# TinyMPC/tinympc-matlab

Hardware: AMD Instinct MI355X
Metric: ADMM iterations/s, batched quadrotor nx=12 nu=4 N=50 (instance-iterations/s, whole job) (higher is better)
Workload: dtype f64

## Files before the change

### __graft_entry__.py

```python
from __future__ import annotations

import hashlib
import importlib.util
import os
import re
import shutil
import subprocess
import sys

ROOT = os.path.dirname(os.path.abspath(__file__))
if ROOT not in sys.path:
    sys.path.insert(0, ROOT)
PKG_DIR = os.path.join(ROOT, "tinympc-matlab_amd")
PKG_NAME = "tinympc_matlab_amd"
CSRC = os.path.join(PKG_DIR, "csrc")
HIP_LIB = os.path.join(PKG_DIR, "libtinympc_hip.so")
ORACLE_DIR = os.path.join(ROOT, "oracle")
REFERENCE_SRC = "/root/reference/src/codegen_src"

HIP_SOURCES = ["tinympc_kernels.hip", "tinympc_precompute_rows.hip", "tinympc_solve.hip", "tinympc_solve_b.hip", "tinympc_solve_fam.hip", "tinympc_solve_adapt.hip", "tinympc_imod_a.hip", "tinympc_solve_c.hip", "tinympc_solve_d.hip", "tinympc_solve_dr.hip", "tinympc_lean_d.hip", "tinympc_lstart_d.hip", "tinympc_ltrim_d.hip", "tinympc_solve_dw.hip", "tinympc_solve_dx.hip", "tinympc_jit.hip", "tinympc_solve_m.hip", "tinympc_precompute_large.hip", "tinympc_handle.hip", "tinympc_plan.hip", "tinympc_session.hip", "tinympc_capi.hip",
               "tinympc_codegen.hip"]
HIP_LINTED = ["tinympc_precompute_rows.hip", "tinympc_solve.hip", "tinympc_solve_b.hip", "tinympc_solve_fam.hip", "tinympc_solve_adapt.hip", "tinympc_imod_a.hip",
              "tinympc_solve_c.hip", "tinympc_solve_d.hip", "tinympc_solve_dr.hip", "tinympc_lean_d.hip", "tinympc_lstart_d.hip", "tinympc_ltrim_d.hip", "tinympc_solve_dw.hip", "tinympc_solve_dx.hip"]
JIT_EMBEDDED = ["tinympc_device.h", "tinympc_sweep.h", "tinympc_fam_red.h", "tinympc_solve_d_chain.h", "tinympc_solve_dw_chain.h", "tinympc_solve_dx_chain.h",
                "tinympc_solve_e_common.h", "tinympc_solve_dwide.h", "tinympc_solve_d.hip", "tinympc_solve_dw.hip", "tinympc_solve_dx.hip", "tinympc_solve_e.hip",
                "tinympc_solve_f.hip"]
_ROCKET = ["-DTINY_JIT_NX=6", "-DTINY_JIT_NU=3", "-DTINY_JIT_N=100", "-DTINY_JIT_CT=0", "-DTINY_JIT_FAM=1"]
_ROCKET_FAM = ["-DTINY_JIT_E_NROUND=1", "-DTINY_JIT_E_NCONE=2", "-DTINY_JIT_E_CONES={0,0,2},{0,6,8}", "-DTINY_JIT_E_NLX=1", "-DTINY_JIT_E_NLU=0"]
HIP_BUILTINS = [
    ("k_builtin_e_rocket100", "tinympc_solve_e.hip",
     _ROCKET + ["-DTINY_JIT_E_WPG=8", "-DTINY_JIT_E_WPS=2", "-DTINY_JIT_E_S=13"] + _ROCKET_FAM +
     ["-DTINY_JIT_E_GC_LDS=0", "-DTINY_JIT_E_GL_LDS=0", "-DTINY_JIT_E_LX_LDS=0", "-DTINY_JIT_E_KFAM=1", "-DTINY_JIT_E_DREG=1"]),
    ("k_builtin_f_rocket100", "tinympc_solve_f.hip", _ROCKET + ["-DTINY_JIT_F_WPG=4", "-DTINY_JIT_F_S=7"] + _ROCKET_FAM + ["-DTINY_JIT_F_KFAM=1"]),
    ("k_builtin_f_rocket100_session", "tinympc_solve_f.hip", _ROCKET + ["-DTINY_JIT_F_WPG=4", "-DTINY_JIT_F_S=7"] + _ROCKET_FAM + ["-DTINY_JIT_F_KFAM=1", "-DTINY_JIT_F_SESSION=1"]),
]
_NO_FAM = ["-DTINY_JIT_E_NROUND=0", "-DTINY_JIT_E_NCONE=0", "-DTINY_JIT_E_CONES={-1,0,0}", "-DTINY_JIT_E_NLX=0", "-DTINY_JIT_E_NLU=0"]
for _name, _nx, _nu, _N, _wpg, _S in (("cartpole20", 4, 1, 20, 2, 3), ("quadrotor50", 12, 4, 50, 4, 4)):
    for _suffix, _ct, _extra in (("", 1, []), ("_var", 0, []), ("_session", 0, ["-DTINY_JIT_F_SESSION=1"])):
        HIP_BUILTINS.append(("k_builtin_f_%s%s" % (_name, _suffix), "tinympc_solve_f.hip",
                             ["-DTINY_JIT_NX=%d" % _nx, "-DTINY_JIT_NU=%d" % _nu, "-DTINY_JIT_N=%d" % _N, "-DTINY_JIT_CT=%d" % _ct, "-DTINY_JIT_FAM=0",
                              "-DTINY_JIT_F_WPG=%d" % _wpg, "-DTINY_JIT_F_S=%d" % _S] + _NO_FAM + _extra))
HIP_BUILTINS_D = [("k_builtin_d_quadrotor50_models", "tinympc_solve_d.hip",
                   ["-DTINY_JIT_NX=12", "-DTINY_JIT_NU=4", "-DTINY_JIT_N=50", "-DTINY_JIT_VREG=49", "-DTINY_JIT_WPS=1", "-DTINY_JIT_WPG=4",
                    "-DTINY_JIT_CT=1", "-DTINY_JIT_FAM=0", "-DTINY_JIT_ADAPT=0", "-DTINY_JIT_IMOD=1"])]
ALL_BUILTINS = HIP_BUILTINS + HIP_BUILTINS_D
BUILD_DIR = os.path.join(ROOT, "build", "hip")
HIP_CFLAGS = ["--offload-arch=gfx950", "-O3", "-std=c++17", "-fPIC", "-fno-gpu-rdc",
              "-Wall", "-Wno-unused-function", "-I" + os.path.join(ROOT, "include"), "-I" + CSRC, "-I" + BUILD_DIR]
HIP_LDFLAGS = ["--offload-arch=gfx950", "-shared", "-fPIC", "-fno-gpu-rdc", "-lhiprtc"]


def load_package():
    if PKG_NAME in sys.modules:
        return sys.modules[PKG_NAME]
    spec = importlib.util.spec_from_file_location(
        PKG_NAME, os.path.join(PKG_DIR, "__init__.py"), submodule_search_locations=[PKG_DIR])
# ... 292 lines not shown
```

### tinympc-matlab_amd/csrc/tinympc_device.h

```cpp
#pragma once
#ifndef __HIPCC_RTC__
#include <hip/hip_runtime.h>
#endif

namespace tinympc {

__host__ __device__ inline size_t ops_doubles(int W, int KT) { return (size_t)2 * W * KT + 3 * W; }

__host__ __device__ inline size_t table_rows(int N) { return (size_t)N + 2; }

constexpr int V_PAD = 4;
__host__ __device__ inline size_t v_rows(int N) { return (size_t)N + 1 + 2 * V_PAD; }
__host__ __device__ inline size_t tables_doubles(int W, int N) { return 3 * table_rows(N) * W + W; }

#if defined(__HIPCC__) || defined(__HIPCC_RTC__)
__device__ __forceinline__ void host_store(double *p, double v) { __hip_atomic_store(p, v, __ATOMIC_RELAXED, __HIP_MEMORY_SCOPE_SYSTEM); }
#endif

struct PrecomputeParams {
    int nx, nu;
    double rho;
    const double *A, *B, *fdyn, *Qd, *Rd;
    double *Kinf, *Pinf, *Quu_inv, *AmBKt, *APf, *BPf;
    int *info;
// ... 250 lines not shown
    double *zero;
    size_t zero_doubles;
    double *xmin, *xmax, *umin, *umax;
    size_t X, U;
    double inf;
    double *rho_inst;
    int batch;
    double rho;
    double *mail;
};
hipError_t launch_setup_init(const SetupInitParams &p, hipStream_t stream);
hipError_t launch_fill_bounds(double *xmin, double *xmax, size_t X, double *umin, double *umax, size_t U, double inf, hipStream_t stream);
hipError_t launch_reset_stats(int *istats, double *dstats, double *rho_inst, int batch, double rho, hipStream_t stream);
size_t lqr_scratch_doubles(int nx, int nu);
size_t precompute_large_scratch_doubles(int nx, int nu);
hipError_t launch_precompute_large(const PrecomputeParams &p, hipStream_t stream);
hipError_t launch_build_operators(const OperatorParams &p, hipStream_t stream);
hipError_t launch_build_tables(const TableParams &p, hipStream_t stream);
hipError_t launch_store_inst_refs(const InstRefStoreParams &p, hipStream_t stream);
hipError_t launch_build_inst_tables(const InstTableParams &p, hipStream_t stream);
hipError_t launch_fill_inst_models(const InstModelFillParams &p, hipStream_t stream);
hipError_t launch_store_inst_diag(const InstDiagParams &p, hipStream_t stream);
enum class SolveExt { Box, Families, Adaptive, InstRefs, InstBounds, InstModels };
hipError_t launch_solve_a(const SolveParams &p, SolveExt ext, int W, int KT, size_t lds_bytes, hipStream_t stream);
hipError_t launch_solve_b(const SolveParams &p, int W, int KT, size_t lds_bytes, hipStream_t stream);
size_t solve_b_lds_bytes(int nx, int nu, int N, int W);
constexpr int WAVES_PER_GROUP_B = 4;
bool solve_d_supported(int nx, int nu, int N, bool const_tables);
hipError_t launch_solve_d(const SolveParams &p, hipStream_t stream);
hipError_t launch_solve_d_refill(const SolveParams &p, hipStream_t stream);
hipError_t launch_solve_d_lean(const SolveParams &p, hipStream_t stream);
hipError_t launch_solve_d_lean_start(const SolveParams &p, hipStream_t stream);
hipError_t launch_solve_d_lean_trim(const SolveParams &p, hipStream_t stream);
int solve_d_workgroups(int nu, int N, bool const_tables, int groups);
size_t solve_d_lds_bytes(int nu, int N, bool const_tables);
int solve_d_resident_workgroups(int wpg);
int solve_d_wavefronts_per_workgroup(int nu, int N, bool const_tables);
bool solve_dw_supported(int nx, int nu, int N, bool const_tables);
hipError_t launch_solve_dw(const SolveParams &p, hipStream_t stream);
int solve_dw_workgroups(int nu, int N, int groups);
size_t solve_dw_lds_bytes(int nu, int N);
bool solve_dx_supported(int nx, int nu, int N, bool const_tables);
hipError_t launch_solve_dx(const SolveParams &p, hipStream_t stream);
int solve_dx_workgroups(int nu, int N, int groups);
size_t solve_dx_lds_bytes(int nu, int N);
hipError_t launch_solve_c(const SolveParams &p, int W, int KT, size_t lds_bytes, hipStream_t stream);
hipError_t launch_build_chunk_tables(const ChunkTableParams &p, hipStream_t stream);
size_t f_input_table_doubles(int nu, int S);
hipError_t launch_build_f_input_tables(const ChunkTableParams &p, hipStream_t stream);
void chunk_plan(int N, int *S, int *C, int *Lc);
size_t solve_c_lds_bytes(int nx, int Lc);
size_t solve_c_lds_bytes_refs(int nx, int nu, int N, int Lc);
size_t chunk_table_doubles(int nx, int Lc);
int chunk_ks(int nx);
hipError_t launch_build_adapt(const AdaptTableParams &p, hipStream_t stream);
inline hipError_t ensure_dynamic_lds(const void *fn, size_t bytes, size_t (&cache)[16]) {
    int dev = 0;
    hipError_t e = hipGetDevice(&dev);
    if (e != hipSuccess) return e;
    if (dev >= 0 && dev < 16 && cache[dev] >= bytes) return hipSuccess;
    e = hipFuncSetAttribute(fn, hipFuncAttributeMaxDynamicSharedMemorySize, (int)bytes);
    if (e == hipSuccess && dev >= 0 && dev < 16) cache[dev] = bytes;
    return e;
}

bool solve_m_supported(int nx, int nu);
// ... 32 lines not shown
```

### tinympc-matlab_amd/csrc/tinympc_plan.hip

```cpp
#include <cstring>
#include "tinympc_handle.h"

using namespace tinympc;
using namespace tinympc::host;

namespace {

void arm_completion_flag(tinympc_solver *s, SolveParams &p) {
    if (!p.host_sol) return;
    s->session_seq += 1;
    p.host_seq = (double)s->session_seq;
    s->flag_pending = true;
}

void decide_layout_d_variants(tinympc_solver *s) {
    if (!s->layout_d) return;
    if (s->d_varying < 0 && !s->tables_const()) {
        if (s->W == 16 && !s->d_jit && solve_d_supported(s->nx, s->nu, s->N, false)) {
            s->d_varying = 1;
        } else {
            s->d_varying_jit = solve_jit_supported(s->W, s->nx, s->nu, s->N, false);
            s->d_varying = s->d_varying_jit ? 1 : 0;
        }
    }
// ... 205 lines not shown
    const bool ct = s->tables_const();
    long resident;
    if (jit) resident = solve_jit_resident_wavefronts(s->W, s->nx, s->nu, s->N, ct);
    else {
        const int wpg = solve_d_wavefronts_per_workgroup(s->nu, s->N, ct);
        resident = (long)solve_d_resident_workgroups(wpg) * wpg;
    }
    const bool reachable = s->st.abs_pri_tol > 0.0 && s->st.abs_dua_tol > 0.0;
    if ((long)s->groups <= resident) return false;
    if (!reachable && mode != 1) return false;
    return !jit || solve_jit_refill_supported(s->W, s->nx, s->nu, s->N, ct);
}

static bool lean_applies(const tinympc_solver *s, const LaunchPlan &pl) {
    if (pl.kernel != KernelId::D_COMPILED || s->W != 16 || pl.adaptive || pl.families || s->zero_copy_tick || s->st.max_iter <= 0)
        return false;
    if (pl.inst_models) return false;
    if (refill_applies(s, pl)) return false;
    const char *env = getenv("TINYMPC_LEAN");
    const int mode = env ? atoi(env) : -1;
    if (mode == 0) return false;
    if (mode == 1) return true;
    const bool reachable = s->st.abs_pri_tol > 0.0 && s->st.abs_dua_tol > 0.0;
    return s->st.check_termination != 1 || !reachable;
}
static bool lean_start_applies() {
    const char *env = getenv("TINYMPC_LEAN_START");
    return !env || atoi(env) != 0;
}
static bool lean_trim_applies() {
    const char *env = getenv("TINYMPC_LEAN_TRIM");
    return lean_start_applies() && (!env || atoi(env) != 0);
}
static const char *lean_words(const tinympc_solver *s, const LaunchPlan &pl) {
    return !lean_applies(s, pl) ? "" : lean_trim_applies() ? " lean lds-start trim" : lean_start_applies() ? " lean lds-start" : " lean";
}

int launch(tinympc_solver *s, bool timed) {
    int rc;
    s->flag_pending = false;
    if ((rc = resolve_plan(s))) return rc;
    const LaunchPlan pl = current_plan(s);
    const bool fam = pl.families, adaptive = pl.adaptive;
    if (s->inst_tables() && !pl.inst_refs) {
        const bool r = s->inst.refs(), b = s->inst.bounds, m = s->inst.models;
        const char *what[3], *back[3];
        int n = 0;
        if (r) { what[n] = "per-instance references (set_x_ref_batch / set_u_ref_batch)"; back[n++] = "tinympc_set_x_ref / tinympc_set_u_ref return to shared references"; }
        if (b) { what[n] = "per-instance bounds (set_bound_constraints_batch)"; back[n++] = "tinympc_set_bound_constraints returns to shared bounds"; }
        if (m) { what[n] = "per-instance models (set_model_batch)"; back[n++] = "tinympc_clear_model_batch returns to the shared model"; }
        std::string subj, way;
        for (int i = 0; i < n; ++i) {
            subj += std::string(i == 0 ? "" : i == n - 1 ? " and " : ", ") + what[i];
            way += std::string(i == 0 ? "" : ", ") + back[i];
        }
        return fail(TINYMPC_ERR_UNSUPPORTED, "%s are not supported %s; %s", subj.c_str(),
                    s->layout_m ? "for systems with nx+nu > 64" : fam ? "with cone / linear constraint families" : "with adaptive rho", way.c_str());
    }
    if (s->refs_on_host && (adaptive || pl.inst_models)) {
        if ((rc = flush_host_refs(s))) return rc;
    }
    if ((rc = refresh_derived(s))) return rc;
    if (adaptive && fam)
        return fail(TINYMPC_ERR_UNSUPPORTED, "adaptive_rho together with cone / linear constraint families is not supported");
    if (s->layout_m && adaptive)
        return fail(TINYMPC_ERR_UNSUPPORTED, "adaptive_rho is not supported for systems with nx+nu > 64");
    if (fam && pl.kernel != KernelId::E && pl.kernel != KernelId::F && pl.kernel != KernelId::M && family_structure(s).beyond_generic())
        return fail(TINYMPC_ERR_UNSUPPORTED, "more than %d linear rows per side, %d cones or %d rounds of overlapping cones run on the run-time "
// ... 54 lines not shown
        p.dXref = s->dXref; p.dUref = s->dUref; p.Pinf = s->dPinf;
        s->refs_on_host = false;
    }
    p.adapt = s->dadapt; p.rho_inst = s->drho_inst;
    if (pl.inst_refs) {
        p.iref_lr = pl.kernel == KernelId::A ? s->inst.lr_rows() : s->inst.lrg;
        p.iref_pn = s->inst.pn;
        if (pl.kernel != KernelId::A) p.ibnd = s->inst.bndg;
        else if (pl.inst_bounds) p.ibnd = s->inst.bnd;
    }
    p.rho_min = s->st.adaptive_rho_min; p.rho_max = s->st.adaptive_rho_max; p.rho_clip = s->st.adaptive_rho_enable_clipping;
    const bool kernel_takes_cold = (pl.kernel == KernelId::D_COMPILED || pl.kernel == KernelId::D_JIT) && s->st.max_iter > 0;
    if (s->cold_state && !kernel_takes_cold && (rc = materialize_cold_state(s))) return rc;
    p.cold = s->cold_state ? 1 : 0;
    s->cold_state = false;
    if (s->st.max_iter > 0) s->sol_zero_pending = false;
    else if ((rc = materialize_zero_solution(s))) return rc;
    if (refill_applies(s, pl) && !p.x0_mirror && !p.u0_host && !p.host_sol) {
        if (!s->drefill && (rc = dalloc(s, &s->drefill, 1))) return rc;
        HIP_TRY(hipMemsetAsync(s->drefill, 0, sizeof(int), s->stream));
        p.refill_next = s->drefill;
    }
    if (timed) HIP_TRY(hipEventRecord(s->ev0, s->stream));
    switch (pl.kernel) {
        case KernelId::M:
            p.ctab = s->dctab;
            HIP_TRY(launch_solve_m(p, s->stream));
            break;
        case KernelId::D_JIT:
            HIP_TRY(launch_solve_jit(p, s->W, s->stream, pl.inst_models));
            break;
        case KernelId::D_COMPILED:
            if (lean_applies(s, pl) && !p.x0_mirror && !p.u0_host && !p.refill_next)
                HIP_TRY(lean_trim_applies()    ? launch_solve_d_lean_trim(p, s->stream)
                        : lean_start_applies() ? launch_solve_d_lean_start(p, s->stream)
                                               : launch_solve_d_lean(p, s->stream));
            else HIP_TRY(s->W == 64 ? launch_solve_dx(p, s->stream) : s->W == 32 ? launch_solve_dw(p, s->stream) : launch_solve_d(p, s->stream));
            break;
        case KernelId::E:
            p.ctab = s->dctab_e; p.chunk_len = s->e_chunk_len; p.chunk_count = s->e_wpg; p.chunk_levels = 1;
            HIP_TRY(launch_solve_e(p, s->fs, s->stream));
            break;
        case KernelId::F:
            p.ctab = s->dctab_f; p.ftab = s->dftab; p.chunk_len = s->f_chunk_len; p.chunk_count = s->f_chunks; p.chunk_levels = 4;
            arm_completion_flag(s, p);
            HIP_TRY(launch_solve_f(p, s->f_fs, s->stream));
            break;
        case KernelId::C:
            p.ctab = s->dctab; p.chunk_len = s->chunk_len; p.chunk_count = s->chunk_count; p.chunk_levels = s->chunk_levels;
            arm_completion_flag(s, p);
            HIP_TRY(launch_solve_c(p, s->W, s->KT, s->lds_bytes_c, s->stream));
            break;
        case KernelId::B:
            HIP_TRY(launch_solve_b(p, s->W, s->KT, s->lds_bytes, s->stream));
            break;
        case KernelId::A:
        case KernelId::FAM_A:
        case KernelId::ADAPT_A: {
            const SolveExt ext = pl.kernel == KernelId::FAM_A ? SolveExt::Families : pl.kernel == KernelId::ADAPT_A ? SolveExt::Adaptive
                                 : pl.inst_models ? SolveExt::InstModels : pl.inst_bounds ? SolveExt::InstBounds : pl.inst_refs ? SolveExt::InstRefs : SolveExt::Box;
            HIP_TRY(launch_solve_a(p, ext, s->W, s->KT, s->lds_bytes_a, s->stream));
            break;
        }
    }
    if (timed) HIP_TRY(hipEventRecord(s->ev1, s->stream));
    return TINYMPC_OK;
}
// ... 77 lines not shown
```

### tinympc-matlab_amd/csrc/tinympc_solve_d.hip

```cpp
#if defined(TINY_BUILTIN) && !defined(TINY_JIT)
#define TINY_JIT 1
#endif
#ifndef TINY_JIT
#include <atomic>
#endif
#include <type_traits>

#include "tinympc_device.h"
#include "tinympc_sweep.h"

#ifndef TINY_REFILL
#if defined(TINY_JIT_REFILL) && TINY_JIT_REFILL
#define TINY_REFILL 1
#else
#define TINY_REFILL 0
#endif
#endif

#ifndef TINY_LEAN
#define TINY_LEAN 0
#endif
#if TINY_LEAN && (TINY_REFILL || defined(TINY_JIT))
#error "TINY_LEAN: compiled-in plain kernels only"
#endif
#ifndef TINY_LEAN_START
#define TINY_LEAN_START 0
#endif
#if TINY_LEAN_START && !TINY_LEAN
#error "TINY_LEAN_START: a variant of the lean kernels"
#endif
#if TINY_LEAN_START && !defined(TINY_LEAN_NO_LDS_START)
#define TINY_LDS_START 1
#else
#define TINY_LDS_START 0
#endif
#if TINY_LEAN_START && !defined(TINY_LEAN_NO_HOIST)
#define TINY_LEAN_HOIST 1
#else
#define TINY_LEAN_HOIST 0
#endif
#ifndef TINY_LEAN_TRIM
#define TINY_LEAN_TRIM 0
#endif
#if TINY_LEAN_TRIM && !(TINY_LEAN_START && TINY_LEAN_HOIST && TINY_LDS_START)
#error "TINY_LEAN_TRIM: a variant of the lean-start kernels (LDS starts and hoisted control)"
#endif
#if TINY_LEAN_TRIM && !defined(TINY_TRIM_NO_DSTORE)
#define TINY_TRIM_DSTORE 1
#define D_DUMP_DOUBLES(nu) (2 * 4 * (nu))
#else
#define TINY_TRIM_DSTORE 0
#endif

#define TINY_STR2(x) #x
#define TINY_STR(x) TINY_STR2(x)
namespace tinympc {
template <int NX, int NU>
struct DStep;
}

#ifdef TINY_JIT
#define D_NX TINY_JIT_NX
#define D_NU TINY_JIT_NU
#include "tinympc_solve_d_chain.h"
#else
#define D_NX 12
#define D_NU 4
#include "tinympc_solve_d_chain.h"
#define D_NX 4
#define D_NU 1
#include "tinympc_solve_d_chain.h"
#endif

namespace tinympc {

template <int I, int E, class F>
__device__ __forceinline__ void static_for(F &&f) {
    if constexpr (I < E) {
        f(std::integral_constant<int, I>{});
        static_for<I + 1, E>(f);
    }
}

constexpr int D_OPS_DOUBLES = 2 * 16 * 16;
// ... 35 lines not shown
    const int want = ns > D_VREG_MAX ? ns - D_VREG_MAX : 0;
    return want <= vlmax ? want : -1;
}
__host__ __device__ constexpr size_t d_lds_bytes(int nu, int N, bool ct, int wpg, int vl, bool fam = false, bool adapt = false, bool imod = false) {
    return sizeof(double) * ((size_t)(imod ? 0 : D_OPS_DOUBLES + D_START_DOUBLES) + (ct ? 0 : d_tab_doubles(N)) + (fam ? D_FAM_DOUBLES : 0) + (adapt ? D_ADAPT_DOUBLES : 0) +
#if TINY_TRIM_DSTORE
                             (size_t)wpg * (vl * 64 + D_DUMP_DOUBLES(nu) + d_d_doubles(nu, N) + (imod ? D_IMOD_WAVE_DOUBLES : 0)));
#else
                             (size_t)wpg * (vl * 64 + d_d_doubles(nu, N) + (imod ? D_IMOD_WAVE_DOUBLES : 0)));
#endif
}

__device__ __forceinline__ unsigned lds_addr(const double *p) { return lds_address(p); }
template <int OFF>
__device__ __forceinline__ double lds_read_async(unsigned addr) {
    return lds_read_issued_here<OFF>(addr);
}
template <int OFF>
__device__ __forceinline__ void lds_write_async(unsigned addr, double v) {
    static_assert(OFF >= 0 && OFF < 65536, "ds offset field is 16 bits");
    asm volatile("ds_write_b64 %0, %1 offset:%2" ::"v"(addr), "v"(v), "n"(OFF) : "memory");
}
template <int OFF>
__device__ __forceinline__ void lds_write_masked(unsigned addr, double v, unsigned long long mask) {
    static_assert(OFF >= 0 && OFF < 65536, "ds offset field is 16 bits");
    unsigned long long saved;
    asm volatile("s_and_saveexec_b64 %[sv], %[m]\n\t"
                 "ds_write_b64 %[a], %[v] offset:%[o]\n\t"
                 "s_mov_b64 exec, %[sv]"
                 : [sv] "=&s"(saved)
                 : [m] "s"(mask), [a] "v"(addr), [v] "v"(v), [o] "n"(OFF)
                 : "memory", "scc");
}
__device__ __forceinline__ void lds_wait() {
    lds_reads_landed();
    asm volatile("" ::: "memory");
}
__device__ __forceinline__ void lds_wait_ops(double (&m)[16]) {
    lds_reads_landed();
#ifdef TINY_D_NO_OPS_WAIT
    asm volatile("" ::: "memory");
#else
    asm volatile(""
                 : "+v"(m[0]), "+v"(m[1]), "+v"(m[2]), "+v"(m[3]), "+v"(m[4]), "+v"(m[5]), "+v"(m[6]), "+v"(m[7]), "+v"(m[8]), "+v"(m[9]),
                   "+v"(m[10]), "+v"(m[11]), "+v"(m[12]), "+v"(m[13]), "+v"(m[14]), "+v"(m[15])
                 :
                 : "memory");
#endif
}

__device__ __forceinline__ bool wave_may_converge_d(unsigned long long bad, unsigned long long live) {
    int any = 0;
#pragma unroll
    for (int j = 0; j < 4; ++j) {
        const unsigned b = (unsigned)(bad >> (j * 16)) & 0xffffu, l = (unsigned)(live >> (j * 16)) & 0xffffu;
        any |= (int)(l != 0u) & (int)(b == 0u);
    }
    return any != 0;
}
#ifdef TINY_D_NO_RARE
#define TINY_RARE(c) (c)
#else
#define TINY_RARE(c) __builtin_expect(!!(c), 0)
#endif

#if TINY_REFILL
// ... 516 lines not shown
#endif
            }
#if TINY_REFILL
            if (TINY_RARE(may) && is_x && active) gV1u[REFILL ? row_offset(cur) : (unsigned)lane] = V0;
#else
            if (TINY_RARE(may) && is_x && active) gV1u[(unsigned)lane] = V0;
#endif
            V0 = snew;
        }
        if constexpr (FAM) {
            double gcn, gln;
            (void)families(x0v, GC0, GL0, gcn, gln);
            if (is_x) {
                GC0 = gcn;
                GL0 = gln;
            }
        }
        double xcur = x0v;
        double dcur = lds_read_async<0>(aD), vcur = 0.0;
#if TINY_LEAN
        if constexpr (VL > 0 && !LEANI) vcur = lds_read_async<0>(aV);
#else
        if constexpr (VL > 0) vcur = lds_read_async<0>(aV);
#endif
        double locur = lo_c, hicur = hi_c;
        if constexpr (!CT) {
            locur = lds_read_async<W * 8>(aT);
            hicur = lds_read_async<(TOFF + W) * 8>(aT);
        }
        lds_wait_ops(m);
#if TINY_LDS_START
        double acur = 0.0;
#endif
        auto fstep = [&](auto S) {
            constexpr int q = decltype(S)::value;
            double dn = 0.0, vn = 0.0, lon = lo_c, hin = hi_c;
            if constexpr (q + 1 < NS) dn = lds_read_async<(q + 1) * DS * 8>(aD);
#if TINY_LEAN
            if constexpr (q + 1 < VL && !LEANI) vn = lds_read_async<(q + 1) * 512>(aV);
#else
            if constexpr (q + 1 < VL) vn = lds_read_async<(q + 1) * 512>(aV);
#endif
            if constexpr (!CT && q + 1 < NS) {
                lon = lds_read_async<(q + 2) * W * 8>(aT);
                hin = lds_read_async<(TOFF + (q + 2) * W) * 8>(aT);
            }
#if TINY_LDS_START
            static_assert(K0, "step 0 starts from c0");
            double an = 0.0;
            if constexpr (LEANI && q + 1 < NS) an = lds_read_issued_here<0>(aC);
#endif
            const double xprev = xcur;
            double snew_q;
#if TINY_LEAN
            if constexpr (LEANI) {
                if constexpr (q >= VL) {
                    if constexpr (K0 && q == 0) xcur = Step::fwd_reg0_nores(dcur, m, c0, locur, hicur, G[q], Vr[q - VL]);
#if TINY_LDS_START
                    else xcur = Step::fwd_reg_start(xcur, dcur, m, acur, locur, hicur, G[q], Vr[q - VL]);
#else
                    else xcur = Step::fwd_reg_nores(xcur, dcur, m, cf, locur, hicur, G[q], Vr[q - VL]);
#endif
                    snew_q = Vr[q - VL];
                } else {
                    double vnew;
                    if constexpr (K0 && q == 0) xcur = Step::fwd_lds0_nores(dcur, m, c0, locur, hicur, G[q], vnew);
#if TINY_LDS_START
                    else xcur = Step::fwd_lds_start(xcur, dcur, m, acur, locur, hicur, G[q], vnew);
#else
                    else xcur = Step::fwd_lds_nores(xcur, dcur, m, cf, locur, hicur, G[q], vnew);
#endif
                    lds_write_async<q * 512>(aV, vnew);
                    snew_q = vnew;
                }
            } else
#endif
            if constexpr (q >= VL) {
                if constexpr (K0 && q == 0) xcur = Step::fwd_reg0(dcur, m, c0, locur, hicur, G[q], Vr[q - VL], pri, dua);
                else xcur = Step::fwd_reg(xcur, dcur, m, cf, locur, hicur, G[q], Vr[q - VL], pri, dua);
                snew_q = Vr[q - VL];
            } else {
                double vnew;
                if constexpr (K0 && q == 0) xcur = Step::fwd_lds0(dcur, m, c0, locur, hicur, G[q], vcur, vnew, pri, dua);
                else xcur = Step::fwd_lds(xcur, dcur, m, cf, locur, hicur, G[q], vcur, vnew, pri, dua);
                lds_write_async<q * 512>(aV, vnew);
                snew_q = vnew;
            }
            if constexpr (ADAPT) {
                if (adapt) {
                    const double gnew = G[q], out = xcur;
                    const double t = group_matvec<W, 16>(mtr, is_x ? gnew : 0.0, 0.0);
                    const double dgx = dgr * (is_x ? xprev : out);
                    const double aty = is_x ? (t - gprev) : (gnew + t);
                    a_dn = fmax(fmax(a_dn, fabs(dgx)), fabs(aty));
                    a_dr = fmax(a_dr, fabs(2.0 * dgx + aty));
                    a_pr = fmax(a_pr, fabs(is_x ? snew_q : (out - snew_q)));
                    a_pn = fmax(fmax(a_pn, fabs(snew_q)), is_x ? 0.0 : fabs(out));
                    gprev = gnew;
                }
            }
            if constexpr (FAM) {
                double gcn, gln;
                const double l = families(xcur, GCr[q], GLr[q], gcn, gln);
                if (row_ok) {
                    GCr[q] = gcn;
                    GLr[q] = gln;
                    LX[q] = l;
                }
            }
            dcur = dn;
            vcur = vn;
#if TINY_LDS_START
            acur = an;
#endif
            if constexpr (!CT) {
                locur = lon;
                hicur = hin;
            }
        };
        constexpr int DF = D_FIRST < NS ? D_FIRST : NS;
        constexpr int NG = 1 + (NS - DF + D_GROUP - 1) / D_GROUP;
        static_for<0, NG>([&](auto Gi) {
            constexpr int s0 = Gi.value == 0 ? 0 : DF + (Gi.value - 1) * D_GROUP;
            constexpr int s1 = Gi.value == 0 ? DF : ((s0 + D_GROUP < NS) ? s0 + D_GROUP : NS);
            if (TINY_RARE(may)) {
                if constexpr (s0 > 0) {
                    if (!adapt) {
                        const bool bad = !((pri < p.abs_pri_tol) && (dua * rho < p.abs_dua_tol));
#if TINY_REFILL
                        may = __builtin_amdgcn_readfirstlane((int)wave_may_converge_d(__ballot(bad), __ballot(REFILL ? chk : active))) != 0;
#else
                        may = __builtin_amdgcn_readfirstlane((int)wave_may_converge_d(__ballot(bad), __ballot(active))) != 0;
#endif
                    }
                }
                if (TINY_RARE(may)) {
#if TINY_REFILL
                    unsigned vo = REFILL ? row_offset(cur) + (unsigned)(koff * 64) : voff;
#else
                    unsigned vo = voff;
#endif
                    double *base = gV1u;
                    asm volatile("" : "+v"(vo), "+s"(base));
                    if (active) static_for<s0, s1>([&](auto S) { (base + S.value * 64)[vo] = vget(S); });
                }
            }
// ... 96 lines not shown
                } else if constexpr (FOLD) {
                    asm("v_add_f64 %[t], %[v1], -%[g1]\n\t"
                        "v_fma_f64 %[px], %[sc], %[t], %[lrT]\n\t"
                        "v_add_f64 %[rn], %[v2], -%[g2]\n\t"
                        "v_fma_f64 %[acc], %[rhom], %[rn], %[lrmc]"
                        : [t] "=&v"(t), [px] "=&v"(px), [acc] "=&v"(acc), [rn] "=&v"(rnext)
                        : [v1] "v"(v1), [g1] "v"(G[NS - 1]), [v2] "v"(v2), [g2] "v"(G[NS - 2]), [sc] "v"(is_x ? nrho : 1.0),
                          [lrT] "v"(is_x ? pnref : 0.0), [rhom] "v"(rhom), [lrmc] "v"(lrmc_f));
                } else {
                    asm("v_add_f64 %[t], %[v1], -%[g1]\n\t"
                        "v_fma_f64 %[px], %[nrho], %[t], %[lrT]\n\t"
                        "v_add_f64 %[t], %[v2], -%[g2]\n\t"
                        "v_fma_f64 %[acc], %[rhom], %[t], %[lrmc]\n\t"
                        "v_fma_f64 %[rn], %[nrho], %[t], %[lr]"
                        : [t] "=&v"(t), [px] "=&v"(px), [acc] "=&v"(acc), [rn] "=&v"(rnext)
                        : [v1] "v"(v1), [g1] "v"(G[NS - 1]), [v2] "v"(v2), [g2] "v"(G[NS - 2]), [nrho] "s"(nrho), [lrT] "v"(lrT),
                          [rhom] "v"(rhom), [lrmc] "v"(lrmc2), [lr] "v"(lr2));
                }
                rcur = px;
            }
            auto vreq = [&](auto S) -> double {
                if constexpr (decltype(S)::value >= VL) return Vr[decltype(S)::value - VL];
                else return lds_read_async<decltype(S)::value * 512>(aV);
            };
            double v2cur = vreq(std::integral_constant<int, (NS >= 3 ? NS - 3 : 0)>{});
            lds_wait_ops(m);
#if TINY_LEAN_HOIST
            if constexpr (LEANI) {
                asm volatile("" : "+v"(G0));
                G0 = G0 - V0;
                asm volatile("" ::"v"(G0));
            }
#endif
            static_for<0, NS - 1>([&](auto I) {
                constexpr int s = NS - 1 - I.value;
                constexpr int s2 = s >= 2 ? s - 2 : 0;
                constexpr int s3 = s >= 3 ? s - 3 : 0;
                double v2n = 0.0;
                if constexpr (s >= 2) v2n = vreq(std::integral_constant<int, s3>{});
                const double lr2 = lr_of(std::integral_constant<int, s2>{});
                const double lrmc2 = is_x ? lr2 + cb : cb;
                double a = acc, an, rn;
                if constexpr (ADAPT) Step::bwd_v(a, px, rcur, m, v2cur, G[s2], rhom_lin, lrmc2, nrho_lin, lr2, an, rn);
                else if constexpr (FOLD) Step::bwd_fold(a, px, rcur, m, v2cur, G[s2], rhom, lrmc_f, an, rn);
                else Step::bwd(a, px, rcur, m, v2cur, G[s2], rhom, lrmc2, nrho, lr2, an, rn);
#if TINY_TRIM_DSTORE
                if constexpr (NO_CTL) lds_write_async<s * DS * 8>(aDw, a);
                else lds_write_masked<s * DS * 8>(aD, a, wr_d);
#else
                lds_write_masked<s * DS * 8>(aD, a, wr_d);
#endif
                px = a;
                rcur = rnext;
                rnext = rn;
                acc = an;
                v2cur = v2n;
            });
            {
                double a = acc;
                Step::bwd_last(a, px, rcur, m);
#if TINY_TRIM_DSTORE
                if constexpr (NO_CTL) lds_write_async<0>(aDw, a);
                else lds_write_masked<0>(aD, a, wr_d);
#else
                lds_write_masked<0>(aD, a, wr_d);
#endif
            }
        }
#if TINY_LEAN
        return false;
    };
    const bool reachable = p.abs_pri_tol > 0.0 && p.abs_dua_tol > 0.0;
    const int last_check = ct > 0 ? (max_iter / ct) * ct : 0;
    for (int it = 0; max_iter > 0;) {
        int nres = max_iter + 1;
        if (ct > 0 && reachable) nres = (it / ct + 1) * ct;
        else if (last_check > it) nres = last_check;
        const int lean_end = __builtin_amdgcn_readfirstlane(nres - 1 < max_iter ? nres - 1 : max_iter);
#if TINY_LEAN_HOIST
        if (it < lean_end) {
            if (iteration(std::integral_constant<int, 2>{}, it)) break;
#if TINY_TRIM_DSTORE
            {
                const unsigned long long live = __ballot(active);
                const unsigned lm = (unsigned)(live & 1ull) | (unsigned)((live >> 15) & 2ull) | (unsigned)((live >> 30) & 4ull) | (unsigned)((live >> 45) & 8ull);
                const int first = __builtin_ctz(lm | 16u);
                const int cls = (r / NU) % 3;
                int jt = cls == 0 ? j : (j ^ 2);
                if (((lm >> jt) & 1u) == 0u) jt = first & 3;
                const unsigned dump = lds_addr(sD) + (unsigned)((jt * NU + r % NU) * 8) - (unsigned)((cls == 2 ? 2 : 1) * DS * 8);
                aDw = (is_u && active) ? aD : dump;
            }
#endif
            for (; it < lean_end; ++it) (void)iteration(std::true_type{}, it);
// ... 32 lines not shown
    }

    const double res_px = group_max<W>(is_x ? snap_pri : 0.0), res_pu = group_max<W>(is_u ? snap_pri : 0.0);
    const double rho_res = ADAPT ? snap_rho : rho;
    const double res_dx = group_max<W>(is_x ? snap_dua : 0.0) * rho_res, res_du = group_max<W>(is_u ? snap_dua : 0.0) * rho_res;

#ifdef TINY_CLOCK_STAMP
    if (p.scratch && lane == 0) {
        unsigned long long *ck = reinterpret_cast<unsigned long long *>(p.scratch) + 8 * (size_t)grp;
        ck[0] = ck_t1 - ck_t0;
        ck[1] = ck_r1 - ck_r0;
        ck[2] = ck_barrier - ck_entry;
        ck[3] = ck_r0 - ck_barrier;
        ck[4] = __builtin_amdgcn_s_memrealtime() - ck_r1;
        ck[5] = ck_entry;
        ck[6] = __builtin_amdgcn_s_memrealtime();
        ck[7] = (unsigned long long)__builtin_amdgcn_s_getreg((31 << 11) | 4) | ((unsigned long long)__builtin_amdgcn_s_getreg((3 << 11) | 20) << 32);
    }
#endif
    if (inst_ok && r == 0) {
        if constexpr (ADAPT) p.rho_inst[inst] = rho;
        p.istats[inst * 2 + 0] = it_done;
        p.istats[inst * 2 + 1] = status;
        if (res_valid) {
            p.dstats[inst * 4 + 0] = res_px;
            p.dstats[inst * 4 + 1] = res_dx;
            p.dstats[inst * 4 + 2] = res_pu;
            p.dstats[inst * 4 + 3] = res_du;
        }
    }
}

#if TINY_LEAN
#if TINY_LEAN_TRIM
#define k_admm_solve_d_lean k_admm_solve_d_lean_trim
#define k_admm_solve_d_gbnd_lean k_admm_solve_d_gbnd_lean_trim
#define launch_solve_d_lean launch_solve_d_lean_trim
static_assert(d_vl(4, 50, true, 4) == 25, "quadrotor N=50: 25 slack slots in LDS with four wavefronts per workgroup");
#elif TINY_LEAN_START
#define k_admm_solve_d_lean k_admm_solve_d_lean_start
#define k_admm_solve_d_gbnd_lean k_admm_solve_d_gbnd_lean_start
#define launch_solve_d_lean launch_solve_d_lean_start
static_assert(d_vl(4, 50, true, 4) == 25, "quadrotor N=50: 25 slack slots in LDS with four wavefronts per workgroup");
#endif
template <int NX, int NU, int N, bool CT, int WPG, int VL>
__global__ void __launch_bounds__(64 * WPG) __attribute__((amdgpu_waves_per_eu(2, 2))) k_admm_solve_d_lean(const SolveParams p) {
    extern __shared__ __attribute__((aligned(16))) double smem[];
    k_admm_solve_d_body<NX, NU, N, CT, WPG, VL>(p, smem);
}
template <int NX, int NU, int N, int WPG, int VL>
__global__ void __launch_bounds__(64 * WPG) __attribute__((amdgpu_waves_per_eu(2, 2))) k_admm_solve_d_gbnd_lean(const SolveParams p) {
    extern __shared__ __attribute__((aligned(16))) double smem[];
    k_admm_solve_d_body<NX, NU, N, true, WPG, VL, false, false, true, false, false, true>(p, smem);
}

__host__ __device__ constexpr int d_wpg(int nu, int N, bool ct) { return d_vl(nu, N, ct, 4) >= 0 ? 4 : 8; }

template <int NX, int NU, int N, bool CT>
static hipError_t launch_d_one(const SolveParams &p, hipStream_t stream) {
    constexpr int WPG = d_wpg(NU, N, CT);
    constexpr int VL = d_vl(NU, N, CT, WPG);
    if constexpr (VL < 0) {
        return hipErrorInvalidValue;
    } else {
        constexpr size_t lds = d_lds_bytes(NU, N, CT, WPG, VL);
        static size_t lds_set_l[16] = {0}, lds_set_lgoal[16] = {0};
        const int wgs = (p.groups + WPG - 1) / WPG;
// ... 230 lines not shown
```

### tinympc-matlab_amd/csrc/tinympc_solve_d_chain.h

```cpp
#if !defined(D_NX) || !defined(D_NU)
#error "define D_NX and D_NU before including tinympc_solve_d_chain.h"
#endif
#if D_NX < 1 || D_NU < 1 || D_NX + D_NU > 16
#error "layout D: 1 <= nx, 1 <= nu, nx + nu <= 16"
#endif

#ifdef TINY_CHAIN_NOALIGN
#define D_AL ""
#define D_MOV64 "v_mov_b64"
#else
#define D_AL ".p2align 3\n\t"
#ifdef TINY_CHAIN_MOV32
#define D_MOV64 "v_mov_b64"
#else
#define D_MOV64 "v_mov_b64_e64"
#endif
#endif
#if (defined(TINY_JIT) && !defined(TINY_BUILTIN)) || defined(TINY_CHAIN_NOP)
#define D_HAZ "s_nop 1\n\t" D_AL
#else
#define D_HAZ D_AL
#endif
#define D_FM_(src, i) "v_fmac_f64_dpp %[a], " src ", %[m" #i "] row_newbcast:" #i " row_mask:0xf bank_mask:0xf\n\t"
#if 0 < D_NX
// ... 269 lines not shown
        asm volatile("v_mov_b64 %[a], %[cf]\n\t" D_HAZ D_CHAIN D_PROJECT_NORES
                     : [a] "=&v"(a), [s] "=&v"(s), [g] "+v"(g), [sn] "+v"(v)
                     : [x] "v"(x), [d] "v"(d), [cf] "v"(cf), [lo] "v"(lo), [hi] "v"(hi), D_MOPS);
        lds_reads_landed();
        return a;
    }
    static __device__ __forceinline__ double fwd_lds_nores(double x, double d, const double (&m)[16], double cf, double lo, double hi, double &g,
                                                           double &vnew) {
        double a, s;
        asm volatile(D_MOV64 " %[a], %[cf]\n\t" D_HAZ D_CHAIN D_PROJECT_NORES
                     : [a] "=&v"(a), [s] "=&v"(s), [g] "+v"(g), [sn] "=&v"(vnew)
                     : [x] "v"(x), [d] "v"(d), [cf] "v"(cf), [lo] "v"(lo), [hi] "v"(hi), D_MOPS);
        lds_reads_landed();
        return a;
    }
    static __device__ __forceinline__ double fwd_reg_start(double x, double d, const double (&m)[16], double a, double lo, double hi, double &g,
                                                           double &v) {
        double s;
        asm volatile(D_HAZ D_CHAIN D_PROJECT_NORES
                     : [a] "+&v"(a), [s] "=&v"(s), [g] "+v"(g), [sn] "+v"(v)
                     : [x] "v"(x), [d] "v"(d), [lo] "v"(lo), [hi] "v"(hi), D_MOPS);
        lds_reads_landed();
        return a;
    }
    static __device__ __forceinline__ double fwd_lds_start(double x, double d, const double (&m)[16], double a, double lo, double hi, double &g,
                                                           double &vnew) {
        double s;
        asm volatile(D_HAZ D_CHAIN D_PROJECT_NORES
                     : [a] "+&v"(a), [s] "=&v"(s), [g] "+v"(g), [sn] "=&v"(vnew)
                     : [x] "v"(x), [d] "v"(d), [lo] "v"(lo), [hi] "v"(hi), D_MOPS);
        lds_reads_landed();
        return a;
    }
    static __device__ __forceinline__ double fwd_reg0_nores(double d, const double (&m)[16], double c0, double lo, double hi, double &g, double &v) {
        double a, s;
        asm volatile("v_mov_b64 %[a], %[cf]\n\t" D_HAZ D_CHAIN_IN D_PROJECT_NORES
                     : [a] "=&v"(a), [s] "=&v"(s), [g] "+v"(g), [sn] "+v"(v)
                     : [d] "v"(d), [cf] "v"(c0), [lo] "v"(lo), [hi] "v"(hi), D_MOPS);
        lds_reads_landed();
        return a;
    }
    static __device__ __forceinline__ double fwd_lds0_nores(double d, const double (&m)[16], double c0, double lo, double hi, double &g, double &vnew) {
        double a, s;
        asm volatile(D_MOV64 " %[a], %[cf]\n\t" D_HAZ D_CHAIN_IN D_PROJECT_NORES
                     : [a] "=&v"(a), [s] "=&v"(s), [g] "+v"(g), [sn] "=&v"(vnew)
                     : [d] "v"(d), [cf] "v"(c0), [lo] "v"(lo), [hi] "v"(hi), D_MOPS);
        lds_reads_landed();
        return a;
    }
    static __device__ __forceinline__ double fwd_reg_woven(double x, double d, const double (&m)[16], double cf, double ap, double lo, double hi,
                                                           double &g, double &v, double &pri, double &dua) {
        double a, s, t, sn;
        asm volatile(D_MOV64 " %[a], %[cf]\n\t" D_HAZ D_CHAIN_WOVEN D_MOV64 " %[v], %[sn]\n\t"
                     : [a] "=&v"(a), [s] "=&v"(s), [t] "=&v"(t), [sn] "=&v"(sn), [g] "+v"(g), [v] "+v"(v), [pri] "+v"(pri), [dua] "+v"(dua)
                     : [x] "v"(x), [d] "v"(d), [cf] "v"(cf), [ap] "v"(ap), [lo] "v"(lo), [hi] "v"(hi), D_MOPS);
        lds_reads_landed();
        return a;
    }
    static __device__ __forceinline__ void project_prev(double ap, double lo, double hi, double &g, double &v, double &pri, double &dua) {
        double s, t, sn;
        asm volatile(D_PROJECT_PREV "v_mov_b64 %[v], %[sn]"
                     : [s] "=&v"(s), [t] "=&v"(t), [sn] "=&v"(sn), [g] "+v"(g), [v] "+v"(v), [pri] "+v"(pri), [dua] "+v"(dua)
                     : [ap] "v"(ap), [lo] "v"(lo), [hi] "v"(hi));
    }
    static __device__ __forceinline__ double fwd_plain(double x, double d, const double (&m)[16], double c) {
        double a;
// ... 115 lines not shown
```

Baseline: 1.177 billion.

## Pair LDS reads across two steps to halve wait points in lean kernel

Adds a paired variant of the trimmed lean layout-D kernel. It issues LDS reads for two upcoming steps at once and waits for landed reads only on every other step, in both the forward and backward sweeps, using new no-wait asm chain variants and plain volatile LDS writes. The goal is to cut the lgkmcnt waits in the serial per-step chain. The cost is more live registers and reliance on careful wait-count ordering. It is enabled by default through an env-gated plan path.

```diff
diff --git a/__graft_entry__.py b/__graft_entry__.py
--- a/__graft_entry__.py
+++ b/__graft_entry__.py
@@ -18,10 +18,10 @@
 ORACLE_DIR = os.path.join(ROOT, "oracle")
 REFERENCE_SRC = "/root/reference/src/codegen_src"
 
-HIP_SOURCES = ["tinympc_kernels.hip", "tinympc_precompute_rows.hip", "tinympc_solve.hip", "tinympc_solve_b.hip", "tinympc_solve_fam.hip", "tinympc_solve_adapt.hip", "tinympc_imod_a.hip", "tinympc_solve_c.hip", "tinympc_solve_d.hip", "tinympc_solve_dr.hip", "tinympc_lean_d.hip", "tinympc_lstart_d.hip", "tinympc_ltrim_d.hip", "tinympc_solve_dw.hip", "tinympc_solve_dx.hip", "tinympc_jit.hip", "tinympc_solve_m.hip", "tinympc_precompute_large.hip", "tinympc_handle.hip", "tinympc_plan.hip", "tinympc_session.hip", "tinympc_capi.hip",
+HIP_SOURCES = ["tinympc_kernels.hip", "tinympc_precompute_rows.hip", "tinympc_solve.hip", "tinympc_solve_b.hip", "tinympc_solve_fam.hip", "tinympc_solve_adapt.hip", "tinympc_imod_a.hip", "tinympc_solve_c.hip", "tinympc_solve_d.hip", "tinympc_solve_dr.hip", "tinympc_lean_d.hip", "tinympc_lstart_d.hip", "tinympc_ltrim_d.hip", "tinympc_lpair_d.hip", "tinympc_solve_dw.hip", "tinympc_solve_dx.hip", "tinympc_jit.hip", "tinympc_solve_m.hip", "tinympc_precompute_large.hip", "tinympc_handle.hip", "tinympc_plan.hip", "tinympc_session.hip", "tinympc_capi.hip",
                "tinympc_codegen.hip"]
 HIP_LINTED = ["tinympc_precompute_rows.hip", "tinympc_solve.hip", "tinympc_solve_b.hip", "tinympc_solve_fam.hip", "tinympc_solve_adapt.hip", "tinympc_imod_a.hip",
-              "tinympc_solve_c.hip", "tinympc_solve_d.hip", "tinympc_solve_dr.hip", "tinympc_lean_d.hip", "tinympc_lstart_d.hip", "tinympc_ltrim_d.hip", "tinympc_solve_dw.hip", "tinympc_solve_dx.hip"]
+              "tinympc_solve_c.hip", "tinympc_solve_d.hip", "tinympc_solve_dr.hip", "tinympc_lean_d.hip", "tinympc_lstart_d.hip", "tinympc_ltrim_d.hip", "tinympc_lpair_d.hip", "tinympc_solve_dw.hip", "tinympc_solve_dx.hip"]
 JIT_EMBEDDED = ["tinympc_device.h", "tinympc_sweep.h", "tinympc_fam_red.h", "tinympc_solve_d_chain.h", "tinympc_solve_dw_chain.h", "tinympc_solve_dx_chain.h",
                 "tinympc_solve_e_common.h", "tinympc_solve_dwide.h", "tinympc_solve_d.hip", "tinympc_solve_dw.hip", "tinympc_solve_dx.hip", "tinympc_solve_e.hip",
                 "tinympc_solve_f.hip"]
diff --git a/tinympc-matlab_amd/csrc/tinympc_device.h b/tinympc-matlab_amd/csrc/tinympc_device.h
--- a/tinympc-matlab_amd/csrc/tinympc_device.h
+++ b/tinympc-matlab_amd/csrc/tinympc_device.h
@@ -306,6 +306,7 @@
 hipError_t launch_solve_d_lean(const SolveParams &p, hipStream_t stream);
 hipError_t launch_solve_d_lean_start(const SolveParams &p, hipStream_t stream);
 hipError_t launch_solve_d_lean_trim(const SolveParams &p, hipStream_t stream);
+hipError_t launch_solve_d_lean_pair(const SolveParams &p, hipStream_t stream);
 int solve_d_workgroups(int nu, int N, bool const_tables, int groups);
 size_t solve_d_lds_bytes(int nu, int N, bool const_tables);
 int solve_d_resident_workgroups(int wpg);
diff --git a/tinympc-matlab_amd/csrc/tinympc_lpair_d.hip b/tinympc-matlab_amd/csrc/tinympc_lpair_d.hip
--- /dev/null
+++ b/tinympc-matlab_amd/csrc/tinympc_lpair_d.hip
@@ -0,0 +1,5 @@
+#define TINY_LEAN 1
+#define TINY_LEAN_START 1
+#define TINY_LEAN_TRIM 1
+#define TINY_LEAN_PAIR 1
+#include "tinympc_solve_d.hip"
diff --git a/tinympc-matlab_amd/csrc/tinympc_plan.hip b/tinympc-matlab_amd/csrc/tinympc_plan.hip
--- a/tinympc-matlab_amd/csrc/tinympc_plan.hip
+++ b/tinympc-matlab_amd/csrc/tinympc_plan.hip
@@ -261,8 +261,16 @@
     const char *env = getenv("TINYMPC_LEAN_TRIM");
     return lean_start_applies() && (!env || atoi(env) != 0);
 }
+static bool lean_pair_applies() {
+    const char *env = getenv("TINYMPC_LEAN_PAIR");
+    return lean_trim_applies() && (!env || atoi(env) != 0);
+}
 static const char *lean_words(const tinympc_solver *s, const LaunchPlan &pl) {
-    return !lean_applies(s, pl) ? "" : lean_trim_applies() ? " lean lds-start trim" : lean_start_applies() ? " lean lds-start" : " lean";
+    return !lean_applies(s, pl)  ? ""
+           : lean_pair_applies() ? " lean lds-start trim pair"
+           : lean_trim_applies() ? " lean lds-start trim"
+           : lean_start_applies() ? " lean lds-start"
+                                  : " lean";
 }
 
 int launch(tinympc_solver *s, bool timed) {
@@ -383,7 +391,8 @@
             break;
         case KernelId::D_COMPILED:
             if (lean_applies(s, pl) && !p.x0_mirror && !p.u0_host && !p.refill_next)
-                HIP_TRY(lean_trim_applies()    ? launch_solve_d_lean_trim(p, s->stream)
+                HIP_TRY(lean_pair_applies()    ? launch_solve_d_lean_pair(p, s->stream)
+                        : lean_trim_applies()  ? launch_solve_d_lean_trim(p, s->stream)
                         : lean_start_applies() ? launch_solve_d_lean_start(p, s->stream)
                                                : launch_solve_d_lean(p, s->stream));
             else HIP_TRY(s->W == 64 ? launch_solve_dx(p, s->stream) : s->W == 32 ? launch_solve_dw(p, s->stream) : launch_solve_d(p, s->stream));
diff --git a/tinympc-matlab_amd/csrc/tinympc_solve_d.hip b/tinympc-matlab_amd/csrc/tinympc_solve_d.hip
--- a/tinympc-matlab_amd/csrc/tinympc_solve_d.hip
+++ b/tinympc-matlab_amd/csrc/tinympc_solve_d.hip
@@ -50,6 +50,17 @@
 #define D_DUMP_DOUBLES(nu) (2 * 4 * (nu))
 #else
 #define TINY_TRIM_DSTORE 0
+#endif
+#ifndef TINY_LEAN_PAIR
+#define TINY_LEAN_PAIR 0
+#endif
+#if TINY_LEAN_PAIR && !(TINY_LEAN_TRIM && TINY_TRIM_DSTORE)
+#error "TINY_LEAN_PAIR: a variant of the trimmed lean kernels"
+#endif
+#if TINY_LEAN_PAIR && !defined(TINY_PAIR_NO_TWOSTEP)
+#define TINY_PAIR_TWOSTEP 1
+#else
+#define TINY_PAIR_TWOSTEP 0
 #endif
 
 #define TINY_STR2(x) #x
@@ -151,6 +162,13 @@
                  : [m] "s"(mask), [a] "v"(addr), [v] "v"(v), [o] "n"(OFF)
                  : "memory", "scc");
 }
+#if TINY_PAIR_TWOSTEP
+template <int OFF>
+__device__ __forceinline__ void lds_write_here(unsigned addr, double v) {
+    static_assert(OFF >= 0 && OFF < 65536 && OFF % 8 == 0, "ds offset field is 16 bits");
+    *((volatile lds_double_as3 *)(size_t)addr + OFF / 8) = v;
+}
+#endif
 __device__ __forceinline__ void lds_wait() {
     lds_reads_landed();
     asm volatile("" ::: "memory");
@@ -733,10 +751,28 @@
 #if TINY_LDS_START
         double acur = 0.0;
 #endif
+#if TINY_PAIR_TWOSTEP
+        constexpr bool PAIRED = LEANI && CT;
+        double dnx = 0.0, anx = 0.0;
+#endif
         auto fstep = [&](auto S) {
             constexpr int q = decltype(S)::value;
             double dn = 0.0, vn = 0.0, lon = lo_c, hin = hi_c;
+#if TINY_PAIR_TWOSTEP
+            constexpr bool LEAD = q % 2 == 0;
+            constexpr bool WAITS = !PAIRED || LEAD || q + 2 >= NS;
+            double dn2 = 0.0, an2 = 0.0;
+            if constexpr (!PAIRED) {
+                if constexpr (q + 1 < NS) dn = lds_read_async<(q + 1) * DS * 8>(aD);
+            } else if constexpr (LEAD) {
+                if constexpr (q + 1 < NS) dn = lds_read_async<(q + 1) * DS * 8>(aD);
+                if constexpr (q + 2 < NS) dn2 = lds_read_async<(q + 2) * DS * 8>(aD);
+            } else {
+                dn = dnx;
+            }
+#else
             if constexpr (q + 1 < NS) dn = lds_read_async<(q + 1) * DS * 8>(aD);
+#endif
 #if TINY_LEAN
             if constexpr (q + 1 < VL && !LEANI) vn = lds_read_async<(q + 1) * 512>(aV);
 #else
@@ -749,7 +785,18 @@
 #if TINY_LDS_START
             static_assert(K0, "step 0 starts from c0");
             double an = 0.0;
+#if TINY_PAIR_TWOSTEP
+            if constexpr (!PAIRED) {
+                if constexpr (LEANI && q + 1 < NS) an = lds_read_issued_here<0>(aC);
+            } else if constexpr (LEAD) {
+                if constexpr (q + 1 < NS) an = lds_read_issued_here<0>(aC);
+                if constexpr (q + 2 < NS) an2 = lds_read_issued_here<0>(aC);
+            } else {
+                an = anx;
+            }
+#else
             if constexpr (LEANI && q + 1 < NS) an = lds_read_issued_here<0>(aC);
+#endif
 #endif
             const double xprev = xcur;
             double snew_q;
@@ -757,6 +804,9 @@
             if constexpr (LEANI) {
                 if constexpr (q >= VL) {
                     if constexpr (K0 && q == 0) xcur = Step::fwd_reg0_nores(dcur, m, c0, locur, hicur, G[q], Vr[q - VL]);
+#if TINY_PAIR_TWOSTEP
+                    else if constexpr (!WAITS) xcur = Step::fwd_reg_start_nw(xcur, dcur, m, acur, locur, hicur, G[q], Vr[q - VL]);
+#endif
 #if TINY_LDS_START
                     else xcur = Step::fwd_reg_start(xcur, dcur, m, acur, locur, hicur, G[q], Vr[q - VL]);
 #else
@@ -766,12 +816,20 @@
                 } else {
                     double vnew;
                     if constexpr (K0 && q == 0) xcur = Step::fwd_lds0_nores(dcur, m, c0, locur, hicur, G[q], vnew);
+#if TINY_PAIR_TWOSTEP
+                    else if constexpr (!WAITS) xcur = Step::fwd_lds_start_nw(xcur, dcur, m, acur, locur, hicur, G[q], vnew);
+#endif
 #if TINY_LDS_START
                     else xcur = Step::fwd_lds_start(xcur, dcur, m, acur, locur, hicur, G[q], vnew);
 #else
                     else xcur = Step::fwd_lds_nores(xcur, dcur, m, cf, locur, hicur, G[q], vnew);
 #endif
+#if TINY_PAIR_TWOSTEP
+                    if constexpr (PAIRED) lds_write_here<q * 512>(aV, vnew);
+                    else lds_write_async<q * 512>(aV, vnew);
+#else
                     lds_write_async<q * 512>(aV, vnew);
+#endif
                     snew_q = vnew;
                 }
             } else
@@ -813,6 +871,12 @@
             vcur = vn;
 #if TINY_LDS_START
             acur = an;
+#endif
+#if TINY_PAIR_TWOSTEP
+            if constexpr (PAIRED && LEAD) {
+                dnx = dn2;
+                anx = an2;
+            }
 #endif
             if constexpr (!CT) {
                 locur = lon;
@@ -975,19 +1039,45 @@
                 asm volatile("" ::"v"(G0));
             }
 #endif
+#if TINY_PAIR_TWOSTEP
+            constexpr bool PAIRED_B = NO_CTL && FOLD;
+            double v2nx = 0.0;
+#endif
             static_for<0, NS - 1>([&](auto I) {
                 constexpr int s = NS - 1 - I.value;
                 constexpr int s2 = s >= 2 ? s - 2 : 0;
                 constexpr int s3 = s >= 3 ? s - 3 : 0;
                 double v2n = 0.0;
+#if TINY_PAIR_TWOSTEP
+                constexpr bool IN_LDS = s >= 2 && s3 < VL, NEXT_IN_LDS = s >= 3 && (s >= 4 ? s - 4 : 0) < VL;
+                constexpr int SL = VL + 2 < NS - 1 ? VL + 2 : NS - 1;
+                constexpr bool LEAD_B = IN_LDS && (SL - s) % 2 == 0;
+                constexpr bool WAITS_B = !PAIRED_B || LEAD_B;
+                if constexpr (!PAIRED_B || !IN_LDS) {
+                    if constexpr (s >= 2) v2n = vreq(std::integral_constant<int, s3>{});
+                } else if constexpr (LEAD_B) {
+                    v2n = vreq(std::integral_constant<int, s3>{});
+                    if constexpr (NEXT_IN_LDS) v2nx = vreq(std::integral_constant<int, (s >= 4 ? s - 4 : 0)>{});
+                } else {
+                    v2n = v2nx;
+                }
+#else
                 if constexpr (s >= 2) v2n = vreq(std::integral_constant<int, s3>{});
+#endif
                 const double lr2 = lr_of(std::integral_constant<int, s2>{});
                 const double lrmc2 = is_x ? lr2 + cb : cb;
                 double a = acc, an, rn;
                 if constexpr (ADAPT) Step::bwd_v(a, px, rcur, m, v2cur, G[s2], rhom_lin, lrmc2, nrho_lin, lr2, an, rn);
+#if TINY_PAIR_TWOSTEP
+                else if constexpr (FOLD && !WAITS_B) Step::bwd_fold_nw(a, px, rcur, m, v2cur, G[s2], rhom, lrmc_f, an, rn);
+#endif
                 else if constexpr (FOLD) Step::bwd_fold(a, px, rcur, m, v2cur, G[s2], rhom, lrmc_f, an, rn);
                 else Step::bwd(a, px, rcur, m, v2cur, G[s2], rhom, lrmc2, nrho, lr2, an, rn);
-#if TINY_TRIM_DSTORE
+#if TINY_PAIR_TWOSTEP
+                if constexpr (PAIRED_B) lds_write_here<s * DS * 8>(aDw, a);
+                else if constexpr (NO_CTL) lds_write_async<s * DS * 8>(aDw, a);
+                else lds_write_masked<s * DS * 8>(aD, a, wr_d);
+#elif TINY_TRIM_DSTORE
                 if constexpr (NO_CTL) lds_write_async<s * DS * 8>(aDw, a);
                 else lds_write_masked<s * DS * 8>(aD, a, wr_d);
 #else
@@ -1001,8 +1091,17 @@
             });
             {
                 double a = acc;
+#if TINY_PAIR_TWOSTEP
+                if constexpr (PAIRED_B) Step::bwd_last_nw(a, px, rcur, m);
+                else Step::bwd_last(a, px, rcur, m);
+#else
                 Step::bwd_last(a, px, rcur, m);
-#if TINY_TRIM_DSTORE
+#endif
+#if TINY_PAIR_TWOSTEP
+                if constexpr (PAIRED_B) lds_write_here<0>(aDw, a);
+                else if constexpr (NO_CTL) lds_write_async<0>(aDw, a);
+                else lds_write_masked<0>(aD, a, wr_d);
+#elif TINY_TRIM_DSTORE
                 if constexpr (NO_CTL) lds_write_async<0>(aDw, a);
                 else lds_write_masked<0>(aD, a, wr_d);
 #else
@@ -1101,7 +1200,12 @@
 }
 
 #if TINY_LEAN
-#if TINY_LEAN_TRIM
+#if TINY_LEAN_PAIR
+#define k_admm_solve_d_lean k_admm_solve_d_lean_pair
+#define k_admm_solve_d_gbnd_lean k_admm_solve_d_gbnd_lean_pair
+#define launch_solve_d_lean launch_solve_d_lean_pair
+static_assert(d_vl(4, 50, true, 4) == 25, "quadrotor N=50: 25 slack slots in LDS with four wavefronts per workgroup");
+#elif TINY_LEAN_TRIM
 #define k_admm_solve_d_lean k_admm_solve_d_lean_trim
 #define k_admm_solve_d_gbnd_lean k_admm_solve_d_gbnd_lean_trim
 #define launch_solve_d_lean launch_solve_d_lean_trim
diff --git a/tinympc-matlab_amd/csrc/tinympc_solve_d_chain.h b/tinympc-matlab_amd/csrc/tinympc_solve_d_chain.h
--- a/tinympc-matlab_amd/csrc/tinympc_solve_d_chain.h
+++ b/tinympc-matlab_amd/csrc/tinympc_solve_d_chain.h
@@ -325,6 +325,35 @@
         lds_reads_landed();
         return a;
     }
+#if TINY_PAIR_TWOSTEP
+    static __device__ __forceinline__ double fwd_reg_start_nw(double x, double d, const double (&m)[16], double a, double lo, double hi, double &g,
+                                                              double &v) {
+        double s;
+        asm volatile(D_HAZ D_CHAIN D_PROJECT_NORES
+                     : [a] "+&v"(a), [s] "=&v"(s), [g] "+v"(g), [sn] "+v"(v)
+                     : [x] "v"(x), [d] "v"(d), [lo] "v"(lo), [hi] "v"(hi), D_MOPS);
+        return a;
+    }
+    static __device__ __forceinline__ double fwd_lds_start_nw(double x, double d, const double (&m)[16], double a, double lo, double hi, double &g,
+                                                              double &vnew) {
+        double s;
+        asm volatile(D_HAZ D_CHAIN D_PROJECT_NORES
+                     : [a] "+&v"(a), [s] "=&v"(s), [g] "+v"(g), [sn] "=&v"(vnew)
+                     : [x] "v"(x), [d] "v"(d), [lo] "v"(lo), [hi] "v"(hi), D_MOPS);
+        return a;
+    }
+    static __device__ __forceinline__ void bwd_fold_nw(double &a, double x, double d, const double (&m)[16], double v2, double g2,
+                                                       double rhom, double lrmc, double &an, double &rn) {
+        asm volatile(D_HAZ D_CHAIN
+                     "v_add_f64 %[t], %[v2], -%[g2]\n\t"
+                     "v_fma_f64 %[an], %[rhom], %[t], %[lrmc]\n\t"
+                     : [a] "+v"(a), [an] "=&v"(an), [t] "=&v"(rn)
+                     : [x] "v"(x), [d] "v"(d), [v2] "v"(v2), [g2] "v"(g2), [rhom] "v"(rhom), [lrmc] "v"(lrmc), D_MOPS);
+    }
+    static __device__ __forceinline__ void bwd_last_nw(double &a, double x, double d, const double (&m)[16]) {
+        asm volatile(D_HAZ D_CHAIN : [a] "+v"(a) : [x] "v"(x), [d] "v"(d), D_MOPS);
+    }
+#endif
     static __device__ __forceinline__ double fwd_reg0_nores(double d, const double (&m)[16], double c0, double lo, double hi, double &g, double &v) {
         double a, s;
         asm volatile("v_mov_b64 %[a], %[cf]\n\t" D_HAZ D_CHAIN_IN D_PROJECT_NORES
```

New measurement: 1.185 billion, median of 6. No clear change (+0.6%).
